# pouyaardehkhani/4DLangSplat

Measured on AMD Instinct MI355X. Metric: rasterizer fwd+bwd frames/sec @ 2M Gaussians, 1352x1014, 32-ch features, higher is better.
Workload: dtype f32; 1 GPU; S2M synthetic (BASELINE configs[2] per GPU; configs[3] batch split); gaussians=2000000, width=1352, height=1014, channels=32, global_batch=8, parallelism=dp1, pipeline=batched, binning=sort, early_views=2, order_on_side=True, num_rendered_mean=5615889

## Files before the change

### 4dlangsplat_amd/csrc/render_bwd_wave.hip

```cpp
#include "lsr_common.h"
#include "lsr_internal.h"
#include "lsr_mfma.h"

namespace lsr {

#ifdef LSR_BWD_STAMPS
__device__ unsigned long long g_bwd_stamps[16];
#define BWD_STAMP(seg)                                                                           \
    do {                                                                                         \
        __builtin_amdgcn_sched_barrier(0);                                                       \
        unsigned long long t_;                                                                   \
        asm volatile("s_memtime %0\n\ts_waitcnt lgkmcnt(0)" : "=s"(t_)::"memory");              \
        __builtin_amdgcn_sched_barrier(0);                                                       \
        if ((seg) > 0) st_sum[(seg) - 1] += t_ - st_prev;                                         \
        st_prev = t_;                                                                            \
    } while (0)
#else
#define BWD_STAMP(seg) do {} while (0)
#endif

constexpr int WG = 16;
constexpr int WFP = 48;
__device__ __forceinline__ int wt_off(int p, int q) { return (p ^ (((p >> 3) & 1) << 2)) * 16 + 4 * (q ^ ((p >> 2) & 3)); }
constexpr int WFIFO = 128;
__device__ __forceinline__ int g_off(int p, int q) { return p * 32 + 8 * (q ^ ((p >> 2) & 3)); }

constexpr int BWD_WAVES = 2;
constexpr int BWD_WAVES_NOL = 3;
template <bool C32, bool PRE, bool NOL>
__global__ void __launch_bounds__(64)
__attribute__((amdgpu_waves_per_eu(NOL ? BWD_WAVES_NOL : BWD_WAVES, NOL ? BWD_WAVES_NOL : BWD_WAVES)))
k_render_bwd_wave(RenderBwdBatch ab) {
    const RenderBwdArgs& a = ab.v[blockIdx.y];
#ifdef LSR_BWD_STAMPS
    unsigned long long st_entry;
    asm volatile("s_memtime %0\n\ts_waitcnt lgkmcnt(0)" : "=s"(st_entry)::"memory");
#endif
    static_assert(!(NOL && C32), "NOL has no language channels");
    __shared__ __attribute__((aligned(16))) __bf16 s_FR[64 * 32];
    __shared__ __attribute__((aligned(16))) __bf16 s_Gh[NOL ? 8 : 64 * 32];
    __shared__ __attribute__((aligned(16))) __bf16 s_Gl[NOL ? 8 : 64 * 32];
    __shared__ __attribute__((aligned(16))) float s_X[WG], s_Y[WG], s_A[WG], s_B[WG], s_C[WG], s_O[WG];
    __shared__ __attribute__((aligned(16))) float s_R[WG], s_Gc[WG], s_Bc[WG], s_D[WG];
    __shared__ uint32_t s_gid[WG];
    __shared__ __attribute__((aligned(16))) uint32_t s_k[WG];
    __shared__ float s_mom[WG][10];
    __shared__ float s_q[WG][17];
    __shared__ float s_lq[WG][36];
    __shared__ uint32_t s_agid[WG];
    __shared__ uint32_t s_fk[WFIFO];
    __shared__ uint32_t s_fg[WFIFO];

    const int b = blockIdx.x;
    const int slot = (b >> 5) * 8 + (b & 7), quad = (b >> 3) & 3;
    if (slot >= a.grid_x * a.grid_y) return;
    const int tile = a.tile_order ? (int)a.tile_order[slot] : slot;
    const int lane = threadIdx.x, g4 = lane >> 4, l16 = lane & 15;
    const int tx = tile % a.grid_x, ty = tile / a.grid_x;
    const int qx0 = tx * LSR_TILE_X + (quad & 1) * 8, qy0 = ty * LSR_TILE_Y + (quad >> 1) * 8;
    const int px = qx0 + (lane & 7), py = qy0 + (lane >> 3);
    const bool inside = px < a.W && py < a.H;
    const size_t HW = (size_t)a.H * a.W, pid = inside ? (size_t)py * a.W + px : 0;
    const uint32_t last_contributor = inside ? a.n_contrib[pid] : 0u;
    uint32_t nrep = last_contributor;
#pragma unroll
    for (int off = 32; off >= 1; off >>= 1) nrep = max(nrep, (uint32_t)__shfl_xor((int)nrep, off));
    nrep = __builtin_amdgcn_readfirstlane(nrep);
    if (nrep == 0) return;
#ifdef LSR_BWD_STAMPS
    unsigned long long st_nrep;
    asm volatile("s_memtime %0\n\ts_waitcnt lgkmcnt(0)" : "=s"(st_nrep)::"memory");
#endif
    const uint2 range = a.ranges[tile];
    const int C = C32 ? 32 : (NOL ? 0 : (a.include_feature ? a.C : 0));
    const float bx0 = (float)qx0, by0 = (float)qy0;

    const float T_final = inside ? a.final_T[pid] : 0.0f;
    float T = T_final;
    float g0 = 0.0f, g1 = 0.0f, g2 = 0.0f, gD = 0.0f;
    if (inside) {
        g0 = a.dL_dcolor[pid]; g1 = a.dL_dcolor[HW + pid]; g2 = a.dL_dcolor[2 * HW + pid];
        if (a.dL_ddepth) gD = a.dL_ddepth[pid];
    }

    bf16x8 bm[2];
    {
        if constexpr (!NOL) {
            float gl[32];
#pragma unroll
            for (int c = 0; c < 32; ++c)
                gl[c] = (inside && a.dL_dlang && c < C) ? a.dL_dlang[(size_t)c * HW + pid] : 0.0f;
#pragma unroll
            for (int c8 = 0; c8 < 4; ++c8) {
                bf16x8 vh, vl;
#pragma unroll
                for (int j = 0; j < 8; ++j) {
                    __bf16 h, l;
                    split_bf16(gl[8 * c8 + j], h, l);
                    vh[j] = h; vl[j] = l;
                }
                *reinterpret_cast<bf16x8*>(s_Gh + g_off(lane, c8)) = vh;
                *reinterpret_cast<bf16x8*>(s_Gl + g_off(lane, c8)) = vl;
            }
        }
        {
            const float x = (float)(lane & 7), y = (float)(lane >> 3);
            const float gv[4] = {g0, g1, g2, gD};
            bf16x8 r0, r1;
            r0[0] = (__bf16)1.0f; r0[1] = (__bf16)x; r0[2] = (__bf16)y;
            r0[3] = (__bf16)(x * x); r0[4] = (__bf16)(x * y); r0[5] = (__bf16)(y * y);
#pragma unroll
            for (int c = 0; c < 4; ++c) {
                __bf16 h, l;
                split_bf16(gv[c], h, l);
                if (c < 2) r0[6 + c] = h; else r1[c - 2] = h;
                r1[2 + c] = l;
            }
            r1[6] = (__bf16)0.0f; r1[7] = (__bf16)0.0f;
            *reinterpret_cast<bf16x8*>(s_FR + lane * 16) = r0;
            *reinterpret_cast<bf16x8*>(s_FR + lane * 16 + 8) = r1;
            wave_lds_sync();
#pragma unroll
            for (int kb = 0; kb < 2; ++kb) {
                const __bf16* p = s_FR + (32 * kb + 8 * g4 + (l16 >> 2)) * 16 + 4 * (l16 & 3);
                bm[kb] = __builtin_shufflevector(ds_read_tr16(p), ds_read_tr16(p + 4 * 16), 0, 1, 2, 3, 4, 5, 6, 7);
            }
            wave_lds_sync();
        }
    }
    auto g_b1 = [&](const __bf16* G, int pb) {
        return *reinterpret_cast<const bf16x8*>(G + g_off(16 * pb + l16, g4));
    };
    auto g_b2 = [&](const __bf16* G, int kb, int nb) {
        const int p = 32 * kb + 8 * g4 + (l16 >> 2), q = 2 * nb + ((l16 & 3) >> 1), o = 4 * (l16 & 1);
        const bf16x4 lo4 = ds_read_tr16(G + g_off(p, q) + o), hi4 = ds_read_tr16(G + g_off(p + 4, q) + o);
        return __builtin_shufflevector(lo4, hi4, 0, 1, 2, 3, 4, 5, 6, 7);
    };
    __bf16* s_Fh = s_FR;
    __bf16* s_Fl = s_FR + WG * WFP;
    __bf16* s_Rh = s_FR;
    __bf16* s_Rl = s_FR + 64 * 16;

    const float bg_dot = a.bg[0] * g0 + a.bg[1] * g1 + a.bg[2] * g2;
    const float bg_term = -T_final * bg_dot;
    const float ddelx_dx = 0.5f * (float)a.W, ddely_dy = 0.5f * (float)a.H;
    float acc_dot = 0.0f, last_dot = 0.0f, last_alpha = 0.0f;
    const float pxf = (float)px, pyf = (float)py;

    int pos = (int)nrep;
    int head = 0, tail = 0;
    uint32_t sc_w = *at32(a.point_list, range.x + max(pos - 64 + lane, 0));
    auto scan_fill = [&](int want) {
        while (tail - head < want && pos > 0) {
            const int k = pos - 64 + lane;
            const uint32_t word = sc_w;
            const uint32_t gid = word & PL_ID_MASK;
            const bool cand = k >= 0 && ((word >> (PL_QUAD_SHIFT + quad)) & 1u);
            const uint64_t m = __ballot(cand);
            if (cand) {
                const int rank = lane == 63 ? 0 : __popcll(m >> (lane + 1));
                const int s = (tail + rank) & (WFIFO - 1);
                s_fk[s] = (uint32_t)k;
                s_fg[s] = gid;
            }
            tail += __popcll(m);
            pos = max(pos - 64, 0);
            sc_w = *at32(a.point_list, range.x + max(k - 64, 0));
        }
        wave_lds_sync();
    };
    struct Pf {
        uint32_t gid, k;
        float2 xy;
        float4 co, rgbd, f0, f1;
    };
    auto load_group = [&](Pf& pf, int n) __attribute__((always_inline)) {
        {
            const bool ok = lane < n;
            const int s = (head + lane) & (WFIFO - 1);
            pf.gid = ok ? s_fg[s] : 0u;
            pf.k = ok ? s_fk[s] : 0xFFFFFFFFu;
            pf.xy = *at32(a.xy, pf.gid);
            pf.co = *at32(a.conic_o, pf.gid);
            pf.rgbd = *at32(a.rgbd, pf.gid);
        }
        const int e = lane >> 2, c0 = 8 * (lane & 3);
        const uint32_t gid = e < n ? s_fg[(head + e) & (WFIFO - 1)] : 0u;
        if constexpr (NOL) {
            (void)gid; (void)c0;
        } else if constexpr (C32) {
            if constexpr (PRE) {
                const uint4* q = reinterpret_cast<const uint4*>(a.lang_split);
                pf.f0 = __builtin_bit_cast(float4, *at32(q, gid * 8u + (uint32_t)(c0 >> 3)));
                pf.f1 = __builtin_bit_cast(float4, *at32(q, gid * 8u + 4u + (uint32_t)(c0 >> 3)));
            } else {
                const float4* r = reinterpret_cast<const float4*>(at32(a.lang, gid * 32u + c0));
                pf.f0 = r[0];
                pf.f1 = r[1];
            }
        } else {
            float f[8];
#pragma unroll
            for (int j = 0; j < 8; ++j) f[j] = (c0 + j < C) ? *at32(a.lang, gid * (uint32_t)C + c0 + j) : 0.0f;
            pf.f0 = make_float4(f[0], f[1], f[2], f[3]);
            pf.f1 = make_float4(f[4], f[5], f[6], f[7]);
        }
        head += n;
    };
    auto store_group = [&](const Pf& pf) __attribute__((always_inline)) {
        if (lane < WG) {
            s_gid[lane] = pf.gid;
            s_k[lane] = pf.k;
            s_X[lane] = pf.xy.x; s_Y[lane] = pf.xy.y;
            s_A[lane] = -0.5f * pf.co.x; s_B[lane] = -pf.co.y; s_C[lane] = -0.5f * pf.co.z; s_O[lane] = pf.co.w;
            s_R[lane] = pf.rgbd.x; s_Gc[lane] = pf.rgbd.y; s_Bc[lane] = pf.rgbd.z; s_D[lane] = pf.rgbd.w;
        }
        const int e = lane >> 2, c0 = 8 * (lane & 3);
        if constexpr (NOL) {
            (void)e; (void)c0;
        } else if constexpr (C32 && PRE) {
            *reinterpret_cast<uint4*>(s_Fh + e * WFP + c0) = __builtin_bit_cast(uint4, pf.f0);
            *reinterpret_cast<uint4*>(s_Fl + e * WFP + c0) = __builtin_bit_cast(uint4, pf.f1);
        } else {
            const float f[8] = {pf.f0.x, pf.f0.y, pf.f0.z, pf.f0.w, pf.f1.x, pf.f1.y, pf.f1.z, pf.f1.w};
            bf16x8 h8, l8;
#pragma unroll
            for (int j = 0; j < 8; ++j) {
                __bf16 h, l;
                split_bf16(f[j], h, l);
                h8[j] = h; l8[j] = l;
            }
            *reinterpret_cast<bf16x8*>(s_Fh + e * WFP + c0) = h8;
            *reinterpret_cast<bf16x8*>(s_Fl + e * WFP + c0) = l8;
        }
        wave_lds_sync();
    };

    int acnt = 0;
    auto issue_atomics = [&]() {
        if (acnt == 0) return;
        const int ch = lane & 31, q = lane & 15;
        float lv[WG / 2], sv[WG / 4];
        uint32_t lo[WG / 2], so[WG / 4];
        if constexpr (!NOL) {
#pragma unroll
            for (int j = 0; j < WG / 2; ++j) {
                const int e = (lane >> 5) + 2 * j;
                lv[j] = s_lq[e][ch];
                lo[j] = s_agid[e] * (uint32_t)C + ch;
            }
        }
#pragma unroll
        for (int r = 0; r < WG / 4; ++r) {
            const int e = (lane >> 4) + 4 * r;
            sv[r] = s_q[e][q];
            so[r] = s_agid[e] * (uint32_t)ACC_PITCH + q;
        }
        if (!NOL && a.acc_lang) {
#pragma unroll
            for (int j = 0; j < WG / 2; ++j)
                if ((lane >> 5) + 2 * j < acnt && ch < C && lv[j] != 0.0f) atomicAdd(at32(a.acc_lang, lo[j]), lv[j]);
        }
#pragma unroll
        for (int r = 0; r < WG / 4; ++r)
            if ((lane >> 4) + 4 * r < acnt && q < 10 && sv[r] != 0.0f) atomicAdd(at32(a.acc_small, so[r]), sv[r]);
        acnt = 0;
    };

#ifdef LSR_BWD_STAMPS
    unsigned long long st_scan;
    asm volatile("s_memtime %0\n\ts_waitcnt lgkmcnt(0)" : "=s"(st_scan)::"memory");
#endif
    scan_fill(WG);
    int cnt = min(WG, tail - head);
    Pf pf;
    if (cnt > 0) load_group(pf, cnt);
#ifdef LSR_BWD_STAMPS
    unsigned long long st_sum[8] = {0, 0, 0, 0, 0, 0, 0, 0}, st_prev = 0, st_loop;
    asm volatile("s_memtime %0\n\ts_waitcnt lgkmcnt(0)" : "=s"(st_loop)::"memory");
#endif
    while (cnt > 0) {
        BWD_STAMP(0);
        store_group(pf);
        BWD_STAMP(1);
        scan_fill(WG);
        BWD_STAMP(2);
        issue_atomics();
        BWD_STAMP(3);
        const int next_cnt = min(WG, tail - head);
        if (next_cnt > 0) load_group(pf, next_cnt);
        BWD_STAMP(4);

        float S[WG];
        if constexpr (NOL) {
#pragma unroll
            for (int e = 0; e < WG; ++e) S[e] = 0.0f;
        } else {
            const bf16x8 ah = *reinterpret_cast<const bf16x8*>(s_Fh + l16 * WFP + 8 * g4);
            const bf16x8 al = *reinterpret_cast<const bf16x8*>(s_Fl + l16 * WFP + 8 * g4);
            f32x4 d[4];
#pragma unroll
            for (int pb = 0; pb < 4; ++pb) {
                const bf16x8 bh = g_b1(s_Gh, pb), bl = g_b1(s_Gl, pb);
                d[pb] = f32x4{0.0f, 0.0f, 0.0f, 0.0f};
                d[pb] = LSR_MFMA16(ah, bh, d[pb]);
                d[pb] = LSR_MFMA16(ah, bl, d[pb]);
                d[pb] = LSR_MFMA16(al, bh, d[pb]);
            }
            wave_lds_sync();
#pragma unroll
            for (int i = 0; i < 4; ++i) {
                float x[4] = {d[0][i], d[1][i], d[2][i], d[3][i]};
                transpose_lane_groups(x);
#pragma unroll
                for (int p = 0; p < 4; ++p) S[4 * p + i] = x[p];
            }
        }

        BWD_STAMP(5);
        float wv[WG], tv[WG];
        constexpr int RB = 2;
        const lsr_f2 px2 = {pxf, pxf}, py2 = {pyf, pyf};
        struct PairIn {
            lsr_f2 X, Y, A, B, Cc, O, R, Gc, Bc, D;
            uint2 kk;
        };
        auto ld_pair = [&](int e0) __attribute__((always_inline)) {
            auto ld2 = [&](const float* base) { return *reinterpret_cast<const lsr_f2*>(base + e0); };
            PairIn q;
            q.X = ld2(s_X); q.Y = ld2(s_Y); q.A = ld2(s_A); q.B = ld2(s_B); q.Cc = ld2(s_C); q.O = ld2(s_O);
            q.R = ld2(s_R); q.Gc = ld2(s_Gc); q.Bc = ld2(s_Bc); q.D = ld2(s_D);
            q.kk = *reinterpret_cast<const uint2*>(s_k + e0);
            return q;
        };
        constexpr bool PIPE = !NOL;
        PairIn pin = ld_pair(0);
#pragma unroll
        for (int e0 = 0; e0 < WG; e0 += RB) {
        float Gv[RB], alv[RB], romv[RB], dotv[RB];
        bool act[RB];
        PairIn pnext;
        if constexpr (PIPE) {
            if (e0 + RB < WG) pnext = ld_pair(e0 + RB);
            __builtin_amdgcn_sched_barrier(0);
        } else if (e0 > 0) {
            pin = ld_pair(e0);
        }
        {
            const lsr_f2 X = pin.X, Y = pin.Y, A = pin.A, B = pin.B, Cc = pin.Cc, O = pin.O;
            const uint2 kk = pin.kk;
            const lsr_f2 dx = X - px2, dy = Y - py2;
            const lsr_f2 pw = gauss_power2(A, B, Cc, dx, dy);
            const lsr_f2 ge = expf_repro2(pw);
            const lsr_f2 og = O * ge;
            lsr_f2 dot = pin.R * g0;
            dot = __builtin_elementwise_fma(pin.Gc, lsr_f2{g1, g1}, dot);
            dot = __builtin_elementwise_fma(pin.Bc, lsr_f2{g2, g2}, dot);
            dot = __builtin_elementwise_fma(pin.D, lsr_f2{gD, gD}, dot);
#pragma unroll
            for (int u = 0; u < 2; ++u) {
                const int e = e0 + u;
                const float power = u ? pw.y : pw.x;
                const float al = fminf(0.99f, u ? og.y : og.x);
                act[u] = (u ? kk.y : kk.x) < last_contributor && power <= 0.0f && al >= 1.0f / 255.0f;
                alv[u] = act[u] ? al : 0.0f;
                Gv[u] = u ? ge.y : ge.x;
                romv[u] = __builtin_amdgcn_rcpf(1.0f - alv[u]);
                dotv[u] = (u ? dot.y : dot.x) + S[e];
            }
        }
#pragma unroll
        for (int u = 0; u < RB; ++u) {
            const int e = e0 + u;
            const float alpha = alv[u], rom = romv[u], dot = dotv[u];
            T = T * rom;
            acc_dot = __builtin_fmaf(last_alpha, last_dot - acc_dot, acc_dot);
            last_dot = dot;
            last_alpha = alpha;
            float dL_dalpha = (dot - acc_dot) * T;
            dL_dalpha = __builtin_fmaf(rom, bg_term, dL_dalpha);
            wv[e] = alpha * T;
            tv[e] = act[u] ? Gv[u] * dL_dalpha : 0.0f;
        }
        if constexpr (PIPE) {
            if (e0 + RB < WG) pin = pnext;
        }
        }

        BWD_STAMP(6);
        auto write_rows = [&](const float (&r)[WG]) {
#pragma unroll
            for (int q = 0; q < 4; ++q) {
                bf16x4 h4, l4;
#pragma unroll
                for (int j = 0; j < 4; ++j) {
                    __bf16 h, l;
                    split_bf16(r[4 * q + j], h, l);
                    h4[j] = h; l4[j] = l;
                }
                *reinterpret_cast<bf16x4*>(s_Rh + wt_off(lane, q)) = h4;
                *reinterpret_cast<bf16x4*>(s_Rl + wt_off(lane, q)) = l4;
            }
            wave_lds_sync();
        };
        auto read_a = [&](int kb, bf16x8& ah, bf16x8& al) {
            const int row = 32 * kb + 8 * g4 + (l16 >> 2), o0 = wt_off(row, l16 & 3), o1 = wt_off(row + 4, l16 & 3);
            const bf16x4 h0 = ds_read_tr16(s_Rh + o0), h1 = ds_read_tr16(s_Rh + o1);
            const bf16x4 l0 = ds_read_tr16(s_Rl + o0), l1 = ds_read_tr16(s_Rl + o1);
            ah = __builtin_shufflevector(h0, h1, 0, 1, 2, 3, 4, 5, 6, 7);
            al = __builtin_shufflevector(l0, l1, 0, 1, 2, 3, 4, 5, 6, 7);
        };
        f32x4 dacc[3] = {f32x4{0.0f, 0.0f, 0.0f, 0.0f}, f32x4{0.0f, 0.0f, 0.0f, 0.0f}, f32x4{0.0f, 0.0f, 0.0f, 0.0f}};
        write_rows(wv);
#pragma unroll
        for (int kb = 0; kb < 2; ++kb) {
            bf16x8 ah, al;
            read_a(kb, ah, al);
            if constexpr (!NOL) {
#pragma unroll
                for (int nb = 0; nb < 2; ++nb) {
                    const bf16x8 bh = g_b2(s_Gh, kb, nb), bl = g_b2(s_Gl, kb, nb);
                    dacc[nb] = LSR_MFMA16(ah, bh, dacc[nb]);
                    dacc[nb] = LSR_MFMA16(ah, bl, dacc[nb]);
                    dacc[nb] = LSR_MFMA16(al, bh, dacc[nb]);
                }
            }
            dacc[2] = LSR_MFMA16(ah, bm[kb], dacc[2]);
            dacc[2] = LSR_MFMA16(al, bm[kb], dacc[2]);
        }
        wave_lds_sync();
        f32x4 dmom = f32x4{0.0f, 0.0f, 0.0f, 0.0f};
        write_rows(tv);
#pragma unroll
        for (int kb = 0; kb < 2; ++kb) {
            bf16x8 ah, al;
            read_a(kb, ah, al);
            dmom = LSR_MFMA16(ah, bm[kb], dmom);
            dmom = LSR_MFMA16(al, bm[kb], dmom);
        }
        if (l16 < 6) {
#pragma unroll
            for (int i = 0; i < 4; ++i) s_mom[4 * g4 + i][l16] = dmom[i];
        }
        {
            float v[4];
#pragma unroll
            for (int i = 0; i < 4; ++i) v[i] = dacc[2][i] + __shfl_down(dacc[2][i], 4, 16);
            if (l16 >= 6 && l16 < 10) {
#pragma unroll
                for (int i = 0; i < 4; ++i) s_q[4 * g4 + i][l16 - 6] = v[i];
            }
        }
        BWD_STAMP(7);
        if constexpr (!NOL) {
#pragma unroll
            for (int i = 0; i < 4; ++i)
#pragma unroll
                for (int nb = 0; nb < 2; ++nb) s_lq[4 * g4 + i][16 * nb + l16] = dacc[nb][i];
        }
        if (lane < WG) s_agid[lane] = s_gid[lane];
        wave_lds_sync();
        if (lane < cnt) {
            const int e = lane;
            const float M0 = s_mom[e][0], Mx = s_mom[e][1], My = s_mom[e][2];
            const float Mxx = s_mom[e][3], Mxy = s_mom[e][4], Myy = s_mom[e][5];
            const float2 xy = make_float2(s_X[e], s_Y[e]);
            const float4 co = make_float4(-2.0f * s_A[e], -s_B[e], -2.0f * s_C[e], s_O[e]);
            const float X = xy.x - bx0, Y = xy.y - by0;
            const float Sdx = X * M0 - Mx, Sdy = Y * M0 - My;
            const float Sdxdx = X * X * M0 - 2.0f * X * Mx + Mxx;
            const float Sdxdy = X * Y * M0 - X * My - Y * Mx + Mxy;
            const float Sdydy = Y * Y * M0 - 2.0f * Y * My + Myy;
            s_q[e][4] = -co.w * ddelx_dx * (co.x * Sdx + co.y * Sdy);
            s_q[e][5] = -co.w * ddely_dy * (co.z * Sdy + co.y * Sdx);
            s_q[e][6] = -0.5f * co.w * Sdxdx;
            s_q[e][7] = -0.5f * co.w * Sdxdy;
            s_q[e][8] = -0.5f * co.w * Sdydy;
            s_q[e][9] = M0;
        }
        wave_lds_sync();
        acnt = cnt;
        cnt = next_cnt;
        BWD_STAMP(8);
    }
    issue_atomics();
#ifdef LSR_BWD_STAMPS
    if (lane < 8) {
        unsigned long long v = 0;
#pragma unroll
        for (int k = 0; k < 8; ++k) v = lane == k ? st_sum[k] : v;
        atomicAdd(&g_bwd_stamps[lane], v);
    }
    if (lane == 8) atomicAdd(&g_bwd_stamps[8], 1ull);
    {
        unsigned long long st_end;
        asm volatile("s_memtime %0\n\ts_waitcnt lgkmcnt(0)" : "=s"(st_end)::"memory");
        if (lane == 9) atomicAdd(&g_bwd_stamps[9], st_loop - st_entry);
        if (lane == 10) atomicAdd(&g_bwd_stamps[10], st_end - st_entry);
        if (lane == 11) atomicAdd(&g_bwd_stamps[11], st_nrep - st_entry);
        if (lane == 12) atomicAdd(&g_bwd_stamps[12], st_scan - st_nrep);
        if (lane == 13) atomicAdd(&g_bwd_stamps[13], st_loop - st_scan);
    }
#endif
}

constexpr int ORDER_BUCKETS = 1024;
struct TileOrderBatch {
    const uint32_t* tile_max[LSR_MAX_VIEWS];
    uint32_t* order[LSR_MAX_VIEWS];
};
__global__ void __launch_bounds__(1024) k_tile_order(int ntiles, TileOrderBatch tb) {
    __shared__ uint32_t s_cnt[ORDER_BUCKETS];
    __shared__ uint32_t s_wave[16];
    const uint32_t* __restrict__ tile_max = tb.tile_max[blockIdx.x];
    uint32_t* __restrict__ order = tb.order[blockIdx.x];
    if (!order || !tile_max) return;
    const int tid = threadIdx.x, lane = tid & 63, wave = tid >> 6;
    s_cnt[tid] = 0;
    __syncthreads();
    auto bucket = [&](int t) {
        const uint32_t cost = tile_max[t] >> 1;
        return ORDER_BUCKETS - 1 - (int)min(cost, (uint32_t)ORDER_BUCKETS - 1);
    };
    for (int t = tid; t < ntiles; t += 1024) atomicAdd(&s_cnt[bucket(t)], 1u);
    __syncthreads();
    const uint32_t v = s_cnt[tid];
    uint32_t inc = v;
#pragma unroll
    for (int o = 1; o < 64; o <<= 1) {
        const uint32_t y = __shfl_up(inc, o);
        if (lane >= o) inc += y;
    }
    if (lane == 63) s_wave[wave] = inc;
    __syncthreads();
    uint32_t off = 0;
    for (int w = 0; w < wave; ++w) off += s_wave[w];
    s_cnt[tid] = off + inc - v;
    __syncthreads();
    for (int t = tid; t < ntiles; t += 1024) order[atomicAdd(&s_cnt[bucket(t)], 1u)] = (uint32_t)t;
}

void launch_render_bwd_wave_views(const RenderBwdArgs* a, int n, hipStream_t st) {
    const int ntiles = a[0].grid_x * a[0].grid_y;
    RenderBwdBatch ab{};
    TileOrderBatch tb{};
    bool order = false;
    for (int v = 0; v < n; ++v) {
        ab.v[v] = a[v];
        tb.tile_max[v] = a[v].tile_max_contrib;
        tb.order[v] = a[v].tile_order;
        order = order || a[v].tile_order;
    }
    if (order) {
        for (int v = 0; v < n; ++v)
            if (!a[v].tile_order) { ab.v[v].tile_order = nullptr; tb.order[v] = nullptr; }
        hipLaunchKernelGGL(k_tile_order, dim3(n), dim3(1024), 0, st, ntiles, tb);
    }
    const bool c32 = a[0].include_feature && a[0].C == 32;
    const bool nol = !a[0].include_feature || a[0].C == 0;
    const dim3 grid(((ntiles + 7) / 8) * 32, n);
    if (c32 && a[0].lang_split) hipLaunchKernelGGL((k_render_bwd_wave<true, true, false>), grid, dim3(64), 0, st, ab);
    else if (c32) hipLaunchKernelGGL((k_render_bwd_wave<true, false, false>), grid, dim3(64), 0, st, ab);
    else if (nol) hipLaunchKernelGGL((k_render_bwd_wave<false, false, true>), grid, dim3(64), 0, st, ab);
    else hipLaunchKernelGGL((k_render_bwd_wave<false, false, false>), grid, dim3(64), 0, st, ab);
}

}

#ifdef LSR_BWD_STAMPS
extern "C" int lsr_debug_bwd_stamps(unsigned long long* out14) {
    if (hipMemcpyFromSymbol(out14, HIP_SYMBOL(lsr::g_bwd_stamps), 14 * sizeof(unsigned long long)) != hipSuccess) return 2;
    unsigned long long z[16] = {};
    return hipMemcpyToSymbol(HIP_SYMBOL(lsr::g_bwd_stamps), z, sizeof(z)) == hipSuccess ? 0 : 2;
}
#endif
```

Baseline: 983.0 frames/s.

## Add optional two-deep prefetch pipeline to backward wave kernel loop

Restructures the backward per-group loop into a run_group lambda and adds a compile-time DEPTH option that keeps two prefetched Gaussian groups in flight, so global loads get more latency hiding. The prefetch struct now holds only the FIFO head, and gid/k are re-read from the LDS FIFO at store time, which shrinks the registers held across iterations. The default DEPTH is 1, so by default the main effect is the register-saving change plus the asm barriers on lane indices. DEPTH 2 would raise register pressure and add empty-group iterations.

Measured after the change: 954.3 frames/s. -2.9%, worse.

```diff
diff --git a/4dlangsplat_amd/csrc/render_bwd_wave.hip b/4dlangsplat_amd/csrc/render_bwd_wave.hip
--- a/4dlangsplat_amd/csrc/render_bwd_wave.hip
+++ b/4dlangsplat_amd/csrc/render_bwd_wave.hip
@@ -27,6 +27,10 @@
 
 constexpr int BWD_WAVES = 2;
 constexpr int BWD_WAVES_NOL = 3;
+#ifndef LSR_BWD_DEPTH
+#define LSR_BWD_DEPTH 1
+#endif
+constexpr int bwd_depth(bool nol) { return nol ? 1 : LSR_BWD_DEPTH; }
 template <bool C32, bool PRE, bool NOL>
 __global__ void __launch_bounds__(64)
 __attribute__((amdgpu_waves_per_eu(NOL ? BWD_WAVES_NOL : BWD_WAVES, NOL ? BWD_WAVES_NOL : BWD_WAVES)))
@@ -149,40 +153,46 @@
 
     int pos = (int)nrep;
     int head = 0, tail = 0;
+    constexpr int DEPTH = bwd_depth(NOL);
+    static_assert(DEPTH == 1 || DEPTH == 2, "pipeline depth");
     uint32_t sc_w = *at32(a.point_list, range.x + max(pos - 64 + lane, 0));
-    auto scan_fill = [&](int want) {
-        while (tail - head < want && pos > 0) {
-            const int k = pos - 64 + lane;
-            const uint32_t word = sc_w;
-            const uint32_t gid = word & PL_ID_MASK;
-            const bool cand = k >= 0 && ((word >> (PL_QUAD_SHIFT + quad)) & 1u);
-            const uint64_t m = __ballot(cand);
-            if (cand) {
-                const int rank = lane == 63 ? 0 : __popcll(m >> (lane + 1));
-                const int s = (tail + rank) & (WFIFO - 1);
-                s_fk[s] = (uint32_t)k;
-                s_fg[s] = gid;
-            }
-            tail += __popcll(m);
-            pos = max(pos - 64, 0);
-            sc_w = *at32(a.point_list, range.x + max(k - 64, 0));
+    auto scan_round = [&]() __attribute__((always_inline)) {
+        const int k = pos - 64 + lane;
+        const uint32_t word = sc_w;
+        const uint32_t gid = word & PL_ID_MASK;
+        const bool cand = k >= 0 && ((word >> (PL_QUAD_SHIFT + quad)) & 1u);
+        const uint64_t m = __ballot(cand);
+        if (cand) {
+            const int rank = lane == 63 ? 0 : __popcll(m >> (lane + 1));
+            const int s = (tail + rank) & (WFIFO - 1);
+            s_fk[s] = (uint32_t)k;
+            s_fg[s] = gid;
+        }
+        tail += __popcll(m);
+        pos = max(pos - 64, 0);
+        sc_w = *at32(a.point_list, range.x + max(k - 64, 0));
+    };
+    auto scan_fill = [&](int want) __attribute__((always_inline)) {
+        auto more = [&]() { return tail - head < want && pos > 0; };
+        if (more()) {
+            scan_round();
+            while (more()) scan_round();
         }
         wave_lds_sync();
     };
     struct Pf {
-        uint32_t gid, k;
+        int h;
         float2 xy;
         float4 co, rgbd, f0, f1;
     };
     auto load_group = [&](Pf& pf, int n) __attribute__((always_inline)) {
         {
-            const bool ok = lane < n;
             const int s = (head + lane) & (WFIFO - 1);
-            pf.gid = ok ? s_fg[s] : 0u;
-            pf.k = ok ? s_fk[s] : 0xFFFFFFFFu;
-            pf.xy = *at32(a.xy, pf.gid);
-            pf.co = *at32(a.conic_o, pf.gid);
-            pf.rgbd = *at32(a.rgbd, pf.gid);
+            const uint32_t gid = lane < n ? s_fg[s] : 0u;
+            pf.h = head;
+            pf.xy = *at32(a.xy, gid);
+            pf.co = *at32(a.conic_o, gid);
+            pf.rgbd = *at32(a.rgbd, gid);
         }
         const int e = lane >> 2, c0 = 8 * (lane & 3);
         const uint32_t gid = e < n ? s_fg[(head + e) & (WFIFO - 1)] : 0u;
@@ -207,13 +217,16 @@
         }
         head += n;
     };
-    auto store_group = [&](const Pf& pf) __attribute__((always_inline)) {
+    auto store_group = [&](const Pf& pf, int n) __attribute__((always_inline)) {
         if (lane < WG) {
-            s_gid[lane] = pf.gid;
-            s_k[lane] = pf.k;
-            s_X[lane] = pf.xy.x; s_Y[lane] = pf.xy.y;
-            s_A[lane] = -0.5f * pf.co.x; s_B[lane] = -pf.co.y; s_C[lane] = -0.5f * pf.co.z; s_O[lane] = pf.co.w;
-            s_R[lane] = pf.rgbd.x; s_Gc[lane] = pf.rgbd.y; s_Bc[lane] = pf.rgbd.z; s_D[lane] = pf.rgbd.w;
+            int ln = lane;
+            asm volatile("" : "+v"(ln));
+            const int s = (pf.h + ln) & (WFIFO - 1);
+            s_gid[ln] = ln < n ? s_fg[s] : 0u;
+            s_k[ln] = ln < n ? s_fk[s] : 0xFFFFFFFFu;
+            s_X[ln] = pf.xy.x; s_Y[ln] = pf.xy.y;
+            s_A[ln] = -0.5f * pf.co.x; s_B[ln] = -pf.co.y; s_C[ln] = -0.5f * pf.co.z; s_O[ln] = pf.co.w;
+            s_R[ln] = pf.rgbd.x; s_Gc[ln] = pf.rgbd.y; s_Bc[ln] = pf.rgbd.z; s_D[ln] = pf.rgbd.w;
         }
         const int e = lane >> 2, c0 = 8 * (lane & 3);
         if constexpr (NOL) {
@@ -239,31 +252,33 @@
     int acnt = 0;
     auto issue_atomics = [&]() {
         if (acnt == 0) return;
-        const int ch = lane & 31, q = lane & 15;
+        int ln = lane;
+        asm volatile("" : "+v"(ln));
+        const int ch = ln & 31, q = ln & 15;
         float lv[WG / 2], sv[WG / 4];
         uint32_t lo[WG / 2], so[WG / 4];
         if constexpr (!NOL) {
 #pragma unroll
             for (int j = 0; j < WG / 2; ++j) {
-                const int e = (lane >> 5) + 2 * j;
+                const int e = (ln >> 5) + 2 * j;
                 lv[j] = s_lq[e][ch];
                 lo[j] = s_agid[e] * (uint32_t)C + ch;
             }
         }
 #pragma unroll
         for (int r = 0; r < WG / 4; ++r) {
-            const int e = (lane >> 4) + 4 * r;
+            const int e = (ln >> 4) + 4 * r;
             sv[r] = s_q[e][q];
             so[r] = s_agid[e] * (uint32_t)ACC_PITCH + q;
         }
         if (!NOL && a.acc_lang) {
 #pragma unroll
             for (int j = 0; j < WG / 2; ++j)
-                if ((lane >> 5) + 2 * j < acnt && ch < C && lv[j] != 0.0f) atomicAdd(at32(a.acc_lang, lo[j]), lv[j]);
+                if ((ln >> 5) + 2 * j < acnt && ch < C && lv[j] != 0.0f) atomicAdd(at32(a.acc_lang, lo[j]), lv[j]);
         }
 #pragma unroll
         for (int r = 0; r < WG / 4; ++r)
-            if ((lane >> 4) + 4 * r < acnt && q < 10 && sv[r] != 0.0f) atomicAdd(at32(a.acc_small, so[r]), sv[r]);
+            if ((ln >> 4) + 4 * r < acnt && q < 10 && sv[r] != 0.0f) atomicAdd(at32(a.acc_small, so[r]), sv[r]);
         acnt = 0;
     };
 
@@ -271,217 +286,230 @@
     unsigned long long st_scan;
     asm volatile("s_memtime %0\n\ts_waitcnt lgkmcnt(0)" : "=s"(st_scan)::"memory");
 #endif
-    scan_fill(WG);
-    int cnt = min(WG, tail - head);
-    Pf pf;
-    if (cnt > 0) load_group(pf, cnt);
+    scan_fill(DEPTH * WG);
+    Pf pf_a, pf_b;
+    int cnt_a = min(WG, tail - head), cnt_b = 0;
+    if (DEPTH == 2 || cnt_a > 0) load_group(pf_a, cnt_a);
+    if constexpr (DEPTH == 2) {
+        cnt_b = min(WG, tail - head);
+        load_group(pf_b, cnt_b);
+    }
 #ifdef LSR_BWD_STAMPS
     unsigned long long st_sum[8] = {0, 0, 0, 0, 0, 0, 0, 0}, st_prev = 0, st_loop;
     asm volatile("s_memtime %0\n\ts_waitcnt lgkmcnt(0)" : "=s"(st_loop)::"memory");
 #endif
-    while (cnt > 0) {
+    auto run_group = [&](Pf& pf, int& pcnt) __attribute__((always_inline)) {
+        const int cnt = pcnt;
         BWD_STAMP(0);
-        store_group(pf);
+        store_group(pf, cnt);
         BWD_STAMP(1);
         scan_fill(WG);
         BWD_STAMP(2);
         issue_atomics();
         BWD_STAMP(3);
-        const int next_cnt = min(WG, tail - head);
-        if (next_cnt > 0) load_group(pf, next_cnt);
+        pcnt = min(WG, tail - head);
+        if (DEPTH == 2 || pcnt > 0) load_group(pf, pcnt);
         BWD_STAMP(4);
-
-        float S[WG];
-        if constexpr (NOL) {
-#pragma unroll
-            for (int e = 0; e < WG; ++e) S[e] = 0.0f;
-        } else {
-            const bf16x8 ah = *reinterpret_cast<const bf16x8*>(s_Fh + l16 * WFP + 8 * g4);
-            const bf16x8 al = *reinterpret_cast<const bf16x8*>(s_Fl + l16 * WFP + 8 * g4);
-            f32x4 d[4];
-#pragma unroll
-            for (int pb = 0; pb < 4; ++pb) {
-                const bf16x8 bh = g_b1(s_Gh, pb), bl = g_b1(s_Gl, pb);
-                d[pb] = f32x4{0.0f, 0.0f, 0.0f, 0.0f};
-                d[pb] = LSR_MFMA16(ah, bh, d[pb]);
-                d[pb] = LSR_MFMA16(ah, bl, d[pb]);
-                d[pb] = LSR_MFMA16(al, bh, d[pb]);
+        if (DEPTH == 1 || cnt > 0) {
+            float S[WG];
+            if constexpr (NOL) {
+#pragma unroll
+                for (int e = 0; e < WG; ++e) S[e] = 0.0f;
+            } else {
+                const bf16x8 ah = *reinterpret_cast<const bf16x8*>(s_Fh + l16 * WFP + 8 * g4);
+                const bf16x8 al = *reinterpret_cast<const bf16x8*>(s_Fl + l16 * WFP + 8 * g4);
+                f32x4 d[4];
+#pragma unroll
+                for (int pb = 0; pb < 4; ++pb) {
+                    const bf16x8 bh = g_b1(s_Gh, pb), bl = g_b1(s_Gl, pb);
+                    d[pb] = f32x4{0.0f, 0.0f, 0.0f, 0.0f};
+                    d[pb] = LSR_MFMA16(ah, bh, d[pb]);
+                    d[pb] = LSR_MFMA16(ah, bl, d[pb]);
+                    d[pb] = LSR_MFMA16(al, bh, d[pb]);
+                }
+                wave_lds_sync();
+#pragma unroll
+                for (int i = 0; i < 4; ++i) {
+                    float x[4] = {d[0][i], d[1][i], d[2][i], d[3][i]};
+                    transpose_lane_groups(x);
+#pragma unroll
+                    for (int p = 0; p < 4; ++p) S[4 * p + i] = x[p];
+                }
+            }
+
+            BWD_STAMP(5);
+            float wv[WG], tv[WG];
+            constexpr int RB = 2;
+            const lsr_f2 px2 = {pxf, pxf}, py2 = {pyf, pyf};
+            struct PairIn {
+                lsr_f2 X, Y, A, B, Cc, O, R, Gc, Bc, D;
+                uint2 kk;
+            };
+            auto ld_pair = [&](int e0) __attribute__((always_inline)) {
+                auto ld2 = [&](const float* base) { return *reinterpret_cast<const lsr_f2*>(base + e0); };
+                PairIn q;
+                q.X = ld2(s_X); q.Y = ld2(s_Y); q.A = ld2(s_A); q.B = ld2(s_B); q.Cc = ld2(s_C); q.O = ld2(s_O);
+                q.R = ld2(s_R); q.Gc = ld2(s_Gc); q.Bc = ld2(s_Bc); q.D = ld2(s_D);
+                q.kk = *reinterpret_cast<const uint2*>(s_k + e0);
+                return q;
+            };
+            constexpr bool PIPE = !NOL;
+            PairIn pin = ld_pair(0);
+#pragma unroll
+            for (int e0 = 0; e0 < WG; e0 += RB) {
+            float Gv[RB], alv[RB], romv[RB], dotv[RB];
+            bool act[RB];
+            PairIn pnext;
+            if constexpr (PIPE) {
+                if (e0 + RB < WG) pnext = ld_pair(e0 + RB);
+                __builtin_amdgcn_sched_barrier(0);
+            } else if (e0 > 0) {
+                pin = ld_pair(e0);
+            }
+            {
+                const lsr_f2 X = pin.X, Y = pin.Y, A = pin.A, B = pin.B, Cc = pin.Cc, O = pin.O;
+                const uint2 kk = pin.kk;
+                const lsr_f2 dx = X - px2, dy = Y - py2;
+                const lsr_f2 pw = gauss_power2(A, B, Cc, dx, dy);
+                const lsr_f2 ge = expf_repro2(pw);
+                const lsr_f2 og = O * ge;
+                lsr_f2 dot = pin.R * g0;
+                dot = __builtin_elementwise_fma(pin.Gc, lsr_f2{g1, g1}, dot);
+                dot = __builtin_elementwise_fma(pin.Bc, lsr_f2{g2, g2}, dot);
+                dot = __builtin_elementwise_fma(pin.D, lsr_f2{gD, gD}, dot);
+#pragma unroll
+                for (int u = 0; u < 2; ++u) {
+                    const int e = e0 + u;
+                    const float power = u ? pw.y : pw.x;
+                    const float al = fminf(0.99f, u ? og.y : og.x);
+                    act[u] = (u ? kk.y : kk.x) < last_contributor && power <= 0.0f && al >= 1.0f / 255.0f;
+                    alv[u] = act[u] ? al : 0.0f;
+                    Gv[u] = u ? ge.y : ge.x;
+                    romv[u] = __builtin_amdgcn_rcpf(1.0f - alv[u]);
+                    dotv[u] = (u ? dot.y : dot.x) + S[e];
+                }
+            }
+#pragma unroll
+            for (int u = 0; u < RB; ++u) {
+                const int e = e0 + u;
+                const float alpha = alv[u], rom = romv[u], dot = dotv[u];
+                T = T * rom;
+                acc_dot = __builtin_fmaf(last_alpha, last_dot - acc_dot, acc_dot);
+                last_dot = dot;
+                last_alpha = alpha;
+                float dL_dalpha = (dot - acc_dot) * T;
+                dL_dalpha = __builtin_fmaf(rom, bg_term, dL_dalpha);
+                wv[e] = alpha * T;
+                tv[e] = act[u] ? Gv[u] * dL_dalpha : 0.0f;
+            }
+            if constexpr (PIPE) {
+                if (e0 + RB < WG) pin = pnext;
+            }
+            }
+
+            BWD_STAMP(6);
+            auto write_rows = [&](const float (&r)[WG]) {
+#pragma unroll
+                for (int q = 0; q < 4; ++q) {
+                    bf16x4 h4, l4;
+#pragma unroll
+                    for (int j = 0; j < 4; ++j) {
+                        __bf16 h, l;
+                        split_bf16(r[4 * q + j], h, l);
+                        h4[j] = h; l4[j] = l;
+                    }
+                    *reinterpret_cast<bf16x4*>(s_Rh + wt_off(lane, q)) = h4;
+                    *reinterpret_cast<bf16x4*>(s_Rl + wt_off(lane, q)) = l4;
+                }
+                wave_lds_sync();
+            };
+            auto read_a = [&](int kb, bf16x8& ah, bf16x8& al) {
+                const int row = 32 * kb + 8 * g4 + (l16 >> 2), o0 = wt_off(row, l16 & 3), o1 = wt_off(row + 4, l16 & 3);
+                const bf16x4 h0 = ds_read_tr16(s_Rh + o0), h1 = ds_read_tr16(s_Rh + o1);
+                const bf16x4 l0 = ds_read_tr16(s_Rl + o0), l1 = ds_read_tr16(s_Rl + o1);
+                ah = __builtin_shufflevector(h0, h1, 0, 1, 2, 3, 4, 5, 6, 7);
+                al = __builtin_shufflevector(l0, l1, 0, 1, 2, 3, 4, 5, 6, 7);
+            };
+            f32x4 dacc[3] = {f32x4{0.0f, 0.0f, 0.0f, 0.0f}, f32x4{0.0f, 0.0f, 0.0f, 0.0f}, f32x4{0.0f, 0.0f, 0.0f, 0.0f}};
+            write_rows(wv);
+#pragma unroll
+            for (int kb = 0; kb < 2; ++kb) {
+                bf16x8 ah, al;
+                read_a(kb, ah, al);
+                if constexpr (!NOL) {
+#pragma unroll
+                    for (int nb = 0; nb < 2; ++nb) {
+                        const bf16x8 bh = g_b2(s_Gh, kb, nb), bl = g_b2(s_Gl, kb, nb);
+                        dacc[nb] = LSR_MFMA16(ah, bh, dacc[nb]);
+                        dacc[nb] = LSR_MFMA16(ah, bl, dacc[nb]);
+                        dacc[nb] = LSR_MFMA16(al, bh, dacc[nb]);
+                    }
+                }
+                dacc[2] = LSR_MFMA16(ah, bm[kb], dacc[2]);
+                dacc[2] = LSR_MFMA16(al, bm[kb], dacc[2]);
             }
             wave_lds_sync();
-#pragma unroll
-            for (int i = 0; i < 4; ++i) {
-                float x[4] = {d[0][i], d[1][i], d[2][i], d[3][i]};
-                transpose_lane_groups(x);
-#pragma unroll
-                for (int p = 0; p < 4; ++p) S[4 * p + i] = x[p];
-            }
-        }
-
-        BWD_STAMP(5);
-        float wv[WG], tv[WG];
-        constexpr int RB = 2;
-        const lsr_f2 px2 = {pxf, pxf}, py2 = {pyf, pyf};
-        struct PairIn {
-            lsr_f2 X, Y, A, B, Cc, O, R, Gc, Bc, D;
-            uint2 kk;
-        };
-        auto ld_pair = [&](int e0) __attribute__((always_inline)) {
-            auto ld2 = [&](const float* base) { return *reinterpret_cast<const lsr_f2*>(base + e0); };
-            PairIn q;
-            q.X = ld2(s_X); q.Y = ld2(s_Y); q.A = ld2(s_A); q.B = ld2(s_B); q.Cc = ld2(s_C); q.O = ld2(s_O);
-            q.R = ld2(s_R); q.Gc = ld2(s_Gc); q.Bc = ld2(s_Bc); q.D = ld2(s_D);
-            q.kk = *reinterpret_cast<const uint2*>(s_k + e0);
-            return q;
-        };
-        constexpr bool PIPE = !NOL;
-        PairIn pin = ld_pair(0);
-#pragma unroll
-        for (int e0 = 0; e0 < WG; e0 += RB) {
-        float Gv[RB], alv[RB], romv[RB], dotv[RB];
-        bool act[RB];
-        PairIn pnext;
-        if constexpr (PIPE) {
-            if (e0 + RB < WG) pnext = ld_pair(e0 + RB);
-            __builtin_amdgcn_sched_barrier(0);
-        } else if (e0 > 0) {
-            pin = ld_pair(e0);
-        }
-        {
-            const lsr_f2 X = pin.X, Y = pin.Y, A = pin.A, B = pin.B, Cc = pin.Cc, O = pin.O;
-            const uint2 kk = pin.kk;
-            const lsr_f2 dx = X - px2, dy = Y - py2;
-            const lsr_f2 pw = gauss_power2(A, B, Cc, dx, dy);
-            const lsr_f2 ge = expf_repro2(pw);
-            const lsr_f2 og = O * ge;
-            lsr_f2 dot = pin.R * g0;
-            dot = __builtin_elementwise_fma(pin.Gc, lsr_f2{g1, g1}, dot);
-            dot = __builtin_elementwise_fma(pin.Bc, lsr_f2{g2, g2}, dot);
-            dot = __builtin_elementwise_fma(pin.D, lsr_f2{gD, gD}, dot);
-#pragma unroll
-            for (int u = 0; u < 2; ++u) {
-                const int e = e0 + u;
-                const float power = u ? pw.y : pw.x;
-                const float al = fminf(0.99f, u ? og.y : og.x);
-                act[u] = (u ? kk.y : kk.x) < last_contributor && power <= 0.0f && al >= 1.0f / 255.0f;
-                alv[u] = act[u] ? al : 0.0f;
-                Gv[u] = u ? ge.y : ge.x;
-                romv[u] = __builtin_amdgcn_rcpf(1.0f - alv[u]);
-                dotv[u] = (u ? dot.y : dot.x) + S[e];
-            }
-        }
-#pragma unroll
-        for (int u = 0; u < RB; ++u) {
-            const int e = e0 + u;
-            const float alpha = alv[u], rom = romv[u], dot = dotv[u];
-            T = T * rom;
-            acc_dot = __builtin_fmaf(last_alpha, last_dot - acc_dot, acc_dot);
-            last_dot = dot;
-            last_alpha = alpha;
-            float dL_dalpha = (dot - acc_dot) * T;
-            dL_dalpha = __builtin_fmaf(rom, bg_term, dL_dalpha);
-            wv[e] = alpha * T;
-            tv[e] = act[u] ? Gv[u] * dL_dalpha : 0.0f;
-        }
-        if constexpr (PIPE) {
-            if (e0 + RB < WG) pin = pnext;
-        }
-        }
-
-        BWD_STAMP(6);
-        auto write_rows = [&](const float (&r)[WG]) {
-#pragma unroll
-            for (int q = 0; q < 4; ++q) {
-                bf16x4 h4, l4;
-#pragma unroll
-                for (int j = 0; j < 4; ++j) {
-                    __bf16 h, l;
-                    split_bf16(r[4 * q + j], h, l);
-                    h4[j] = h; l4[j] = l;
+            f32x4 dmom = f32x4{0.0f, 0.0f, 0.0f, 0.0f};
+            write_rows(tv);
+#pragma unroll
+            for (int kb = 0; kb < 2; ++kb) {
+                bf16x8 ah, al;
+                read_a(kb, ah, al);
+                dmom = LSR_MFMA16(ah, bm[kb], dmom);
+                dmom = LSR_MFMA16(al, bm[kb], dmom);
+            }
+            if (l16 < 6) {
+#pragma unroll
+                for (int i = 0; i < 4; ++i) s_mom[4 * g4 + i][l16] = dmom[i];
+            }
+            {
+                float v[4];
+#pragma unroll
+                for (int i = 0; i < 4; ++i) v[i] = dacc[2][i] + __shfl_down(dacc[2][i], 4, 16);
+                if (l16 >= 6 && l16 < 10) {
+#pragma unroll
+                    for (int i = 0; i < 4; ++i) s_q[4 * g4 + i][l16 - 6] = v[i];
                 }
-                *reinterpret_cast<bf16x4*>(s_Rh + wt_off(lane, q)) = h4;
-                *reinterpret_cast<bf16x4*>(s_Rl + wt_off(lane, q)) = l4;
-            }
+            }
+            BWD_STAMP(7);
+            if constexpr (!NOL) {
+#pragma unroll
+                for (int i = 0; i < 4; ++i)
+#pragma unroll
+                    for (int nb = 0; nb < 2; ++nb) s_lq[4 * g4 + i][16 * nb + l16] = dacc[nb][i];
+            }
+            if (lane < WG) s_agid[lane] = s_gid[lane];
             wave_lds_sync();
-        };
-        auto read_a = [&](int kb, bf16x8& ah, bf16x8& al) {
-            const int row = 32 * kb + 8 * g4 + (l16 >> 2), o0 = wt_off(row, l16 & 3), o1 = wt_off(row + 4, l16 & 3);
-            const bf16x4 h0 = ds_read_tr16(s_Rh + o0), h1 = ds_read_tr16(s_Rh + o1);
-            const bf16x4 l0 = ds_read_tr16(s_Rl + o0), l1 = ds_read_tr16(s_Rl + o1);
-            ah = __builtin_shufflevector(h0, h1, 0, 1, 2, 3, 4, 5, 6, 7);
-            al = __builtin_shufflevector(l0, l1, 0, 1, 2, 3, 4, 5, 6, 7);
-        };
-        f32x4 dacc[3] = {f32x4{0.0f, 0.0f, 0.0f, 0.0f}, f32x4{0.0f, 0.0f, 0.0f, 0.0f}, f32x4{0.0f, 0.0f, 0.0f, 0.0f}};
-        write_rows(wv);
-#pragma unroll
-        for (int kb = 0; kb < 2; ++kb) {
-            bf16x8 ah, al;
-            read_a(kb, ah, al);
-            if constexpr (!NOL) {
-#pragma unroll
-                for (int nb = 0; nb < 2; ++nb) {
-                    const bf16x8 bh = g_b2(s_Gh, kb, nb), bl = g_b2(s_Gl, kb, nb);
-                    dacc[nb] = LSR_MFMA16(ah, bh, dacc[nb]);
-                    dacc[nb] = LSR_MFMA16(ah, bl, dacc[nb]);
-                    dacc[nb] = LSR_MFMA16(al, bh, dacc[nb]);
-                }
-            }
-            dacc[2] = LSR_MFMA16(ah, bm[kb], dacc[2]);
-            dacc[2] = LSR_MFMA16(al, bm[kb], dacc[2]);
-        }
-        wave_lds_sync();
-        f32x4 dmom = f32x4{0.0f, 0.0f, 0.0f, 0.0f};
-        write_rows(tv);
-#pragma unroll
-        for (int kb = 0; kb < 2; ++kb) {
-            bf16x8 ah, al;
-            read_a(kb, ah, al);
-            dmom = LSR_MFMA16(ah, bm[kb], dmom);
-            dmom = LSR_MFMA16(al, bm[kb], dmom);
-        }
-        if (l16 < 6) {
-#pragma unroll
-            for (int i = 0; i < 4; ++i) s_mom[4 * g4 + i][l16] = dmom[i];
-        }
-        {
-            float v[4];
-#pragma unroll
-            for (int i = 0; i < 4; ++i) v[i] = dacc[2][i] + __shfl_down(dacc[2][i], 4, 16);
-            if (l16 >= 6 && l16 < 10) {
-#pragma unroll
-                for (int i = 0; i < 4; ++i) s_q[4 * g4 + i][l16 - 6] = v[i];
-            }
-        }
-        BWD_STAMP(7);
-        if constexpr (!NOL) {
-#pragma unroll
-            for (int i = 0; i < 4; ++i)
-#pragma unroll
-                for (int nb = 0; nb < 2; ++nb) s_lq[4 * g4 + i][16 * nb + l16] = dacc[nb][i];
-        }
-        if (lane < WG) s_agid[lane] = s_gid[lane];
-        wave_lds_sync();
-        if (lane < cnt) {
-            const int e = lane;
-            const float M0 = s_mom[e][0], Mx = s_mom[e][1], My = s_mom[e][2];
-            const float Mxx = s_mom[e][3], Mxy = s_mom[e][4], Myy = s_mom[e][5];
-            const float2 xy = make_float2(s_X[e], s_Y[e]);
-            const float4 co = make_float4(-2.0f * s_A[e], -s_B[e], -2.0f * s_C[e], s_O[e]);
-            const float X = xy.x - bx0, Y = xy.y - by0;
-            const float Sdx = X * M0 - Mx, Sdy = Y * M0 - My;
-            const float Sdxdx = X * X * M0 - 2.0f * X * Mx + Mxx;
-            const float Sdxdy = X * Y * M0 - X * My - Y * Mx + Mxy;
-            const float Sdydy = Y * Y * M0 - 2.0f * Y * My + Myy;
-            s_q[e][4] = -co.w * ddelx_dx * (co.x * Sdx + co.y * Sdy);
-            s_q[e][5] = -co.w * ddely_dy * (co.z * Sdy + co.y * Sdx);
-            s_q[e][6] = -0.5f * co.w * Sdxdx;
-            s_q[e][7] = -0.5f * co.w * Sdxdy;
-            s_q[e][8] = -0.5f * co.w * Sdydy;
-            s_q[e][9] = M0;
-        }
-        wave_lds_sync();
+            if (lane < cnt) {
+                const int e = lane;
+                const float M0 = s_mom[e][0], Mx = s_mom[e][1], My = s_mom[e][2];
+                const float Mxx = s_mom[e][3], Mxy = s_mom[e][4], Myy = s_mom[e][5];
+                const float2 xy = make_float2(s_X[e], s_Y[e]);
+                const float4 co = make_float4(-2.0f * s_A[e], -s_B[e], -2.0f * s_C[e], s_O[e]);
+                const float X = xy.x - bx0, Y = xy.y - by0;
+                const float Sdx = X * M0 - Mx, Sdy = Y * M0 - My;
+                const float Sdxdx = X * X * M0 - 2.0f * X * Mx + Mxx;
+                const float Sdxdy = X * Y * M0 - X * My - Y * Mx + Mxy;
+                const float Sdydy = Y * Y * M0 - 2.0f * Y * My + Myy;
+                s_q[e][4] = -co.w * ddelx_dx * (co.x * Sdx + co.y * Sdy);
+                s_q[e][5] = -co.w * ddely_dy * (co.z * Sdy + co.y * Sdx);
+                s_q[e][6] = -0.5f * co.w * Sdxdx;
+                s_q[e][7] = -0.5f * co.w * Sdxdy;
+                s_q[e][8] = -0.5f * co.w * Sdydy;
+                s_q[e][9] = M0;
+            }
+            wave_lds_sync();
+        }
         acnt = cnt;
-        cnt = next_cnt;
         BWD_STAMP(8);
+    };
+    if constexpr (DEPTH == 1) {
+        while (cnt_a > 0) run_group(pf_a, cnt_a);
+    } else {
+        while (cnt_a > 0) {
+            run_group(pf_a, cnt_a);
+            run_group(pf_b, cnt_b);
+        }
     }
     issue_atomics();
 #ifdef LSR_BWD_STAMPS
```
